# abhishekjoshi2/cuGP

Hardware: AMD Instinct MI355X
Metric: GP log-lik+grad evals/sec (N=8192, D=10) (higher is better)
Workload: dtype f64; 1 GPU; gp_loglik_grad_N8192_D10; experts=1, experts_per_gpu=1, overlap=True, full=False

## Files before the change

### cugp_amd/csrc/kernels.hip

```cpp
#include "kernels.h"

#include <hip/hip_runtime.h>
#include <hip/hip_ext.h>

#include <cassert>
#include <cstdlib>

namespace cugp {

typedef double d4 __attribute__((ext_vector_type(4)));
typedef double d2 __attribute__((ext_vector_type(2)));

template <class T>
__device__ __forceinline__ T* GP(T* p)
{
    return (T*)(__attribute__((address_space(1))) T*)(unsigned long long)p;
}

#ifdef CUGP_WGTIMES
constexpr unsigned WGT_CAP = 1u << 19;
__device__ unsigned long long g_wgt[4 * WGT_CAP];
__device__ unsigned g_wgt_n;
struct WgTimer {
    unsigned long long t0, c0, tag;
// ... 31 lines not shown
    __device__ __forceinline__ explicit LaunchStamp(unsigned long long* p_, unsigned every = 1)
        : p((p_ && (every <= 1 || blockIdx.x % every == 0 || blockIdx.x + 64 >= gridDim.x)) ? p_ : nullptr)
    {
        if (p && threadIdx.x == 0 && blockIdx.x < 64 && blockIdx.y == 0)
            __hip_atomic_fetch_min(p, (unsigned long long)__builtin_amdgcn_s_memrealtime(), __ATOMIC_RELAXED, __HIP_MEMORY_SCOPE_AGENT);
    }
    __device__ __forceinline__ ~LaunchStamp()
    {
        if (p && threadIdx.x == 0)
            __hip_atomic_fetch_max(p + STAMP_STRIDE, (unsigned long long)__builtin_amdgcn_s_memrealtime(), __ATOMIC_RELAXED, __HIP_MEMORY_SCOPE_AGENT);
    }
};

#include "cov_device.h"
#include "bcm_grad_device.h"

constexpr int BK = 16;
template <int WM> struct Geo {
    static constexpr int BT = 32 * WM;
    static constexpr int PLANE = BT * 16 + 16;
    static constexpr int OPER = (BK / 2) * PLANE;
    static constexpr int STAGE = 2 * OPER;
    static constexpr int LDS = 2 * STAGE;
};
constexpr int GEMM_LDS = Geo<4>::LDS;

constexpr int MT = 16;
constexpr int MTS = MT * (MT + 1);
constexpr int NMT = TILE / MT;
constexpr int NLT = NMT * (NMT + 1) / 2;
constexpr int POTF2_LDS = (NLT * MTS + TILE) * 8;

template <int WM>
__device__ __forceinline__ int bpos(int R)
{
    const int q = R & (16 * WM - 1);
    return (R - q) + (((q >> 5) * 2 + (q & 1)) * 16) + ((q & 31) >> 1);
}

__device__ __forceinline__ int opaque_tid()
{
    int t = threadIdx.x;
    asm volatile("" : "+v"(t));
    return t;
}

template <int WM>
__device__ __forceinline__ void tile_stage_mma(const char* __restrict__ cur, int abase, int bbase,
                                               d4 (&acc)[WM][WM])
{
    typedef Geo<WM> G;
#pragma unroll
    for (int kk = 0; kk < BK / 4; kk++) {
        double a[WM], b[WM];
#pragma unroll
        for (int m = 0; m < WM; m++) {
            a[m] = *(const double*)(cur + abase + kk * 2 * G::PLANE + m * 256);
            b[m] = *(const double*)(cur + bbase + kk * 2 * G::PLANE + m * 256);
        }
#pragma unroll
        for (int m = 0; m < WM; m++)
#pragma unroll
            for (int n = 0; n < WM; n++)
                acc[m][n] = __builtin_amdgcn_mfma_f64_16x16x4f64(a[m], b[n], acc[m][n], 0, 0, 0);
    }
}

#ifdef CUGP_TILE_STAMPS
__device__ unsigned long long g_tile_stamps[64];
__device__ int g_tile_stamp_on;
#define TILE_STAMP(i)                                                              \
    do {                                                                           \
        if (threadIdx.x == 0 && blockIdx.x == 200) {                               \
            g_tile_stamps[i] = __builtin_readcyclecounter();                       \
            g_tile_stamps[32 + i] = __builtin_amdgcn_s_memrealtime();              \
        }                                                                          \
    } while (0)
#else
#define TILE_STAMP(i)
#endif

template <bool NEGA, int WM>
__device__ __forceinline__ void tile_nt(const double* __restrict__ Ag, int lda, const double* __restrict__ Bg,
                                        int ldb, int kbeg, int kend, d4 (&acc)[WM][WM], char* smem)
{
    typedef Geo<WM> G;
    const int t = opaque_tid();
    const int lane = t & 63, wave = t >> 6;
    const int wr = wave >> 1, wc = wave & 1;

    const int srow = t >> 3, skp = t & 7;
    const double* ag = Ag + (size_t)srow * lda + 2 * skp;
    const double* bg = Bg + (size_t)srow * ldb + 2 * skp;
    d2 ra[WM], rb[WM];
    int wa[WM], wb[WM];
#pragma unroll
    for (int q = 0; q < WM; q++) {
        wa[q] = skp * G::PLANE + (srow + 32 * q) * 16;
        wb[q] = G::OPER + skp * G::PLANE + bpos<WM>(srow + 32 * q) * 16;
    }
    const int fr = lane & 15, fk = lane >> 4;
    const int abase = (fk >> 1) * G::PLANE + (wr * 16 * WM + fr) * 16 + (fk & 1) * 8;
    const int bbase = G::OPER + (fk >> 1) * G::PLANE + (wc * 16 * WM + fr) * 16 + (fk & 1) * 8;

    const int nk = (kend - kbeg) / BK;
    if (nk <= 0) return;

#pragma unroll
    for (int q = 0; q < WM; q++) {
        ra[q] = *(const d2*)(ag + (size_t)(32 * q) * lda + kbeg);
        rb[q] = *(const d2*)(bg + (size_t)(32 * q) * ldb + kbeg);
    }
#pragma unroll
    for (int q = 0; q < WM; q++) {
        *(d2*)(smem + wa[q]) = NEGA ? -ra[q] : ra[q];
        *(d2*)(smem + wb[q]) = rb[q];
    }
    __syncthreads();
#ifdef CUGP_TILE_STAMPS
    if (g_tile_stamp_on) TILE_STAMP(1);
#endif

#define CUGP_STAGE(HALF, MORE, KNEXT)                                                              \
    do {                                                                                           \
        const char* cur_ = smem + (HALF) * G::STAGE;                                               \
        char* nxt_ = smem + (1 - (HALF)) * G::STAGE;                                               \
        const bool more_ = (MORE);                                                                 \
        if (more_) {                                                                               \
            const int k_ = (KNEXT);                                                                \
            _Pragma("unroll") for (int q = 0; q < WM; q++) {                                       \
                ra[q] = *(const d2*)(ag + (size_t)(32 * q) * lda + k_);                            \
                rb[q] = *(const d2*)(bg + (size_t)(32 * q) * ldb + k_);                            \
            }                                                                                      \
        }                                                                                          \
        tile_stage_mma<WM>(cur_, abase, bbase, acc);                                               \
        if (more_) {                                                                               \
            _Pragma("unroll") for (int q = 0; q < WM; q++) {                                       \
                *(d2*)(nxt_ + wa[q]) = NEGA ? -ra[q] : ra[q];                                      \
                *(d2*)(nxt_ + wb[q]) = rb[q];                                                      \
            }                                                                                      \
        }                                                                                          \
        __syncthreads();                                                                           \
    } while (0)

    int kt = 0;
    for (; kt + 1 < nk; kt += 2) {
        CUGP_STAGE(0, true, kbeg + (kt + 1) * BK);
        CUGP_STAGE(1, kt + 2 < nk, kbeg + (kt + 2) * BK);
    }
    if (kt < nk) CUGP_STAGE(0, false, 0);
#undef CUGP_STAGE
}

template <int WM>
__device__ __forceinline__ void acc_zero(d4 (&acc)[WM][WM])
{
#pragma unroll
    for (int m = 0; m < WM; m++)
#pragma unroll
        for (int n = 0; n < WM; n++) acc[m][n] = (d4){0.0, 0.0, 0.0, 0.0};
}

#define ACC_ROW(m, r) (wr * 16 * WM + (m) * 16 + (lane >> 4) + 4 * (r))
#define ACC_COL2(np) (wc * 16 * WM + (np) * 32 + 2 * (lane & 15))

template <bool STREAM = false, int WM>
__device__ __forceinline__ void tile_load(const double* __restrict__ C, int ldc, d4 (&acc)[WM][WM])
{
    const int tid = opaque_tid();
    const int lane = tid & 63, wave = tid >> 6;
    const int wr = wave >> 1, wc = wave & 1;
#pragma unroll
    for (int m = 0; m < WM; m++)
#pragma unroll
        for (int r = 0; r < 4; r++)
#pragma unroll
            for (int np = 0; np < WM / 2; np++) {
                const d2* src = (const d2*)(C + (size_t)ACC_ROW(m, r) * ldc + ACC_COL2(np));
                const d2 v = STREAM ? __builtin_nontemporal_load(src) : *src;
                acc[m][2 * np][r] = v[0];
                acc[m][2 * np + 1][r] = v[1];
            }
}

template <bool STREAM = false, int WM>
__device__ __forceinline__ void tile_store(double* __restrict__ C, int ldc, const d4 (&acc)[WM][WM], double alpha)
{
    const int tid = opaque_tid();
    const int lane = tid & 63, wave = tid >> 6;
    const int wr = wave >> 1, wc = wave & 1;
#pragma unroll
    for (int m = 0; m < WM; m++)
#pragma unroll
        for (int r = 0; r < 4; r++)
#pragma unroll
            for (int np = 0; np < WM / 2; np++)
            {
                d2* dst = (d2*)(C + (size_t)ACC_ROW(m, r) * ldc + ACC_COL2(np));
                const d2 v = (d2){alpha * acc[m][2 * np][r], alpha * acc[m][2 * np + 1][r]};
                if (STREAM) __builtin_nontemporal_store(v, dst);
                else *dst = v;
            }
}

template <int SIGN, int WM>
__device__ __forceinline__ void tile_accum_store(double* __restrict__ C, int ldc, const d4 (&acc)[WM][WM])
{
    const int tid = opaque_tid();
    const int lane = tid & 63, wave = tid >> 6;
    const int wr = wave >> 1, wc = wave & 1;
#pragma unroll
    for (int m = 0; m < WM; m++) {
        d2 v[4][WM / 2];
#pragma unroll
        for (int r = 0; r < 4; r++)
#pragma unroll
            for (int np = 0; np < WM / 2; np++)
                v[r][np] = *(const d2*)(C + (size_t)ACC_ROW(m, r) * ldc + ACC_COL2(np));
#pragma unroll
        for (int r = 0; r < 4; r++)
#pragma unroll
            for (int np = 0; np < WM / 2; np++) {
                d2* dst = (d2*)(C + (size_t)ACC_ROW(m, r) * ldc + ACC_COL2(np));
                if (SIGN > 0) *dst = (d2){v[r][np][0] + acc[m][2 * np][r], v[r][np][1] + acc[m][2 * np + 1][r]};
                else *dst = (d2){v[r][np][0] - acc[m][2 * np][r], v[r][np][1] - acc[m][2 * np + 1][r]};
            }
    }
}

template <int WM>
__device__ __forceinline__ void tile_store_t(double* __restrict__ Ct, int ldc, const d4 (&acc)[WM][WM], double alpha,
                                             char* smem)
{
    constexpr int RH = 16 * WM, BT = 32 * WM;
    constexpr int LPC = RH / 2, CPP = 256 / LPC;
    const int t = threadIdx.x, lane = t & 63, wave = t >> 6;
    const int wr = wave >> 1, wc = wave & 1;
    double* sd = (double*)smem;
#pragma unroll
    for (int h = 0; h < 2; h++) {
        __syncthreads();
        if (wr == h) {
#pragma unroll
            for (int m = 0; m < WM; m++)
#pragma unroll
                for (int n = 0; n < WM; n++)
#pragma unroll
                    for (int r = 0; r < 4; r++) {
                        const int col = ACC_COL2(n >> 1) + (n & 1);
                        const int rr = m * 16 + (lane >> 4) + 4 * r;
                        sd[col * RH + (rr ^ ((col >> 1) & 15))] = alpha * acc[m][n][r];
                    }
        }
        __syncthreads();
        const int rr = (t % LPC) * 2;
#pragma unroll
        for (int pass = 0; pass < BT / CPP; pass++) {
            const int col = pass * CPP + t / LPC;
            const int sw = (col >> 1) & 15;
            const d2 v = (d2){sd[col * RH + (rr ^ sw)], sd[col * RH + ((rr + 1) ^ sw)]};
            *(d2*)(Ct + (size_t)col * ldc + h * RH + rr) = v;
        }
    }
}

__device__ __forceinline__ void trap_index(int idx, int wcol, int& ti, int& tj)
{
    const int head = wcol * (wcol + 1) / 2;
    if (idx < head) { tri_index(idx, ti, tj); return; }
    const int rem = idx - head;
    ti = wcol + rem / wcol;
    tj = rem % wcol;
}

template <int WM>
__device__ __forceinline__ void lauum_tile(const double* __restrict__ U, double* __restrict__ Kinv, int ld, int a, int w,
                                           int tile, int sub, char* smem)
{
    constexpr int SUB = 4 / WM, BT = 32 * WM;
    int ti, tj;
    tri_index(tile, ti, tj);
    const int si = (sub / SUB) * BT, sj = (sub % SUB) * BT;
    double* C = Kinv + (size_t)(ti * TILE + si) * ld + tj * TILE + sj;
    d4 acc[WM][WM];
    acc_zero(acc);
    tile_nt<false>(U + (size_t)(ti * TILE + si) * ld, ld, U + (size_t)(tj * TILE + sj) * ld, ld,
                   (ti < a ? a : ti) * TILE, (a + w) * TILE, acc, smem);
    if (ti < a) tile_accum_store<1>(C, ld, acc);
    else tile_store(C, ld, acc, 1.0);
}

// ... 145 lines not shown
    for (int q = 0; q < 2; q++) {
        ra[q] = *(const d2*)(ag + (size_t)(64 * q) * lda + kbeg);
        rb[q] = *(const d2*)(bg + (size_t)(64 * q) * ldb + kbeg);
    }
#pragma unroll
    for (int q = 0; q < 2; q++) {
        *(d2*)(smem + wa[q]) = NEGA ? -ra[q] : ra[q];
        *(d2*)(smem + wb[q]) = rb[q];
    }
    __syncthreads();
#define CUGP_STAGE8(HALF, MORE, KNEXT)                                                              \
    do {                                                                                            \
        const char* cur_ = smem + (HALF) * G::STAGE;                                                \
        char* nxt_ = smem + (1 - (HALF)) * G::STAGE;                                                \
        const bool more_ = (MORE);                                                                  \
        if (more_) {                                                                                \
            const int k_ = (KNEXT);                                                                 \
            _Pragma("unroll") for (int q = 0; q < 2; q++) {                                         \
                ra[q] = *(const d2*)(ag + (size_t)(64 * q) * lda + k_);                             \
                rb[q] = *(const d2*)(bg + (size_t)(64 * q) * ldb + k_);                             \
            }                                                                                       \
        }                                                                                           \
        _Pragma("unroll") for (int kk = 0; kk < BK / 4; kk++) {                                     \
            double a[2], b[4];                                                                      \
            _Pragma("unroll") for (int m = 0; m < 2; m++) a[m] = *(const double*)(cur_ + abase + kk * 2 * G::PLANE + m * 256); \
            _Pragma("unroll") for (int n = 0; n < 4; n++) b[n] = *(const double*)(cur_ + bbase + kk * 2 * G::PLANE + n * 256); \
            _Pragma("unroll") for (int m = 0; m < 2; m++)                                           \
                _Pragma("unroll") for (int n = 0; n < 4; n++)                                       \
                    acc[m][n] = __builtin_amdgcn_mfma_f64_16x16x4f64(a[m], b[n], acc[m][n], 0, 0, 0); \
        }                                                                                           \
        if (more_) {                                                                                \
            _Pragma("unroll") for (int q = 0; q < 2; q++) {                                         \
                *(d2*)(nxt_ + wa[q]) = NEGA ? -ra[q] : ra[q];                                       \
                *(d2*)(nxt_ + wb[q]) = rb[q];                                                       \
            }                                                                                       \
        }                                                                                           \
        __syncthreads();                                                                            \
    } while (0)
    int kt = 0;
    for (; kt + 1 < nk; kt += 2) {
        CUGP_STAGE8(0, true, kbeg + (kt + 1) * BK);
        CUGP_STAGE8(1, kt + 2 < nk, kbeg + (kt + 2) * BK);
    }
    if (kt < nk) CUGP_STAGE8(0, false, 0);
#undef CUGP_STAGE8
}

template <int SIGN>
__device__ __forceinline__ void tile_out8(double* __restrict__ C, int ldc, const d4 (&acc)[2][4])
{
    const int tid = opaque_tid();
    const int lane = tid & 63, wave = tid >> 6;
    const int wr = wave >> 1, wc = wave & 1;
#pragma unroll
    for (int m = 0; m < 2; m++) {
        double* const c0 = C + (size_t)(wr * 32 + m * 16 + (lane >> 4)) * ldc + wc * 64 + 2 * (lane & 15);
        d2 v[4][2];
        if (SIGN != 0) {
#pragma unroll
            for (int r = 0; r < 4; r++)
#pragma unroll
                for (int np = 0; np < 2; np++) v[r][np] = *(const d2*)(c0 + (size_t)(4 * r) * ldc + np * 32);
        }
#pragma unroll
        for (int r = 0; r < 4; r++)
#pragma unroll
            for (int np = 0; np < 2; np++) {
                d2* dst = (d2*)(c0 + (size_t)(4 * r) * ldc + np * 32);
                if (SIGN == 0) *dst = (d2){acc[m][2 * np][r], acc[m][2 * np + 1][r]};
                else if (SIGN > 0) *dst = (d2){v[r][np][0] + acc[m][2 * np][r], v[r][np][1] + acc[m][2 * np + 1][r]};
                else *dst = (d2){v[r][np][0] - acc[m][2 * np][r], v[r][np][1] - acc[m][2 * np + 1][r]};
            }
    }
}

__device__ __forceinline__ void acc_zero8(d4 (&acc)[2][4])
{
#pragma unroll
    for (int m = 0; m < 2; m++)
#pragma unroll
        for (int n = 0; n < 4; n++) acc[m][n] = (d4){0.0, 0.0, 0.0, 0.0};
}

__global__ __launch_bounds__(512, 4) void k_lauum8(const double* __restrict__ U, double* __restrict__ Kinv, int ld, int a,
                                                   int w, const ExpertPtrs* __restrict__ bt, unsigned long long* stamp)
{
    LaunchStamp stamp_(stamp);
    if (bt) { U = GP(bt[blockIdx.y].U); Kinv = GP(bt[blockIdx.y].Kinv); }
    extern __shared__ __attribute__((aligned(16))) char smem[];
    int ti, tj;
    tri_index(blockIdx.x, ti, tj);
    double* C = Kinv + (size_t)(ti * TILE) * ld + tj * TILE;
    d4 acc[2][4];
    acc_zero8(acc);
    tile_nt8<false>(U + (size_t)(ti * TILE) * ld, ld, U + (size_t)(tj * TILE) * ld, ld, (ti < a ? a : ti) * TILE,
                    (a + w) * TILE, acc, smem);
    if (ti < a) tile_out8<1>(C, ld, acc);
    else tile_out8<0>(C, ld, acc);
}

__global__ __launch_bounds__(256, 2) void k_lauum_rest(const double* __restrict__ U, double* __restrict__ Kinv, int ld,
                                                       int a, int w, int x0, const ExpertPtrs* __restrict__ bt)
{
    if (bt) { U = GP(bt[blockIdx.y].U); Kinv = GP(bt[blockIdx.y].Kinv); }
    extern __shared__ __attribute__((aligned(16))) char smem[];
    lauum_tile<2>(U, Kinv, ld, a, w, x0 + (blockIdx.x >> 2), blockIdx.x & 3, smem);
}

__global__ __launch_bounds__(512, 4) void k_trtri_border8(const double* __restrict__ L, double* __restrict__ T,
                                                          const double* __restrict__ U, int ld, int a, int w, int c0,
                                                          int c1, const ExpertPtrs* __restrict__ bt,
                                                          unsigned long long* stamp)
{
    LaunchStamp stamp_(stamp);
    if (bt) { L = GP(bt[blockIdx.y].A); T = GP(bt[blockIdx.y].T); U = GP(bt[blockIdx.y].U); }
    extern __shared__ __attribute__((aligned(16))) char smem[];
    const int tj = blockIdx.x / w, ti = a + blockIdx.x % w;
    double* W = T + (size_t)(tj * TILE) * ld + ti * TILE;
    d4 acc[2][4];
    acc_zero8(acc);
    tile_nt8<false>(U + (size_t)(tj * TILE) * ld, ld, L + (size_t)(ti * TILE) * ld, ld, (tj > c0 ? tj : c0) * TILE,
                    c1 * TILE, acc, smem);
    if (tj < c0) tile_out8<1>(W, ld, acc);
    else tile_out8<0>(W, ld, acc);
}

__global__ __launch_bounds__(256, 2) void k_trtri_border_rest(const double* __restrict__ L, double* __restrict__ T,
                                                              double* __restrict__ U, int ld, int a, int w, int c0,
                                                              int c1, int x0, const ExpertPtrs* __restrict__ bt)
{
    if (bt) { L = GP(bt[blockIdx.y].A); T = GP(bt[blockIdx.y].T); U = GP(bt[blockIdx.y].U); }
    extern __shared__ __attribute__((aligned(16))) char smem[];
    border_tile<2>(L, T, U, ld, a, w, 1, c0, c1, x0 + (blockIdx.x >> 2), blockIdx.x & 3, smem);
}

__global__ __launch_bounds__(256, 2) void k_predict_gemm(const double* __restrict__ Ks, const double* __restrict__ T,
                                                         double* __restrict__ W, int ld, int ntt64, int n64,
                                                         unsigned long long* stamp, const ExpertPtrs* __restrict__ bt)
{
    LaunchStamp stamp_(stamp);
    if (bt) {
        const size_t off = (size_t)blockIdx.y * ntt64 * 64 * ld;
        T = GP(bt[blockIdx.y].T); Ks += off; W += off;
    }
    extern __shared__ __attribute__((aligned(16))) char smem[];
    const int tt = blockIdx.x % ntt64, p = blockIdx.x / ntt64;
#pragma unroll 1
    for (int h = 0; h < 2; h++) {
        const int ti = h == 0 ? n64 - 1 - p : p;
        d4 acc[2][2];
        acc_zero(acc);
        tile_nt<false>(Ks + (size_t)tt * 64 * ld, ld, T + (size_t)ti * 64 * ld, ld, 0, (ti + 1) * 64, acc, smem);
        tile_store(W + (size_t)tt * 64 * ld + ti * 64, ld, acc, 1.0);
    }
}

__global__ __launch_bounds__(256, 2) void k_test_gemm(const double* __restrict__ A, const double* __restrict__ B,
                                                      double* __restrict__ C, int n, int k, int mt)
{
    extern __shared__ __attribute__((aligned(16))) char smem[];
    const int ti = blockIdx.x % mt, tj = blockIdx.x / mt;
    d4 acc[4][4];
    acc_zero(acc);
    tile_nt<false>(A + (size_t)ti * TILE * k, k, B + (size_t)tj * TILE * k, k, 0, k, acc, smem);
    tile_store(C + (size_t)ti * TILE * n + tj * TILE, n, acc, 1.0);
}

__global__ __launch_bounds__(256) void k_mfma_peak(double* sink, int iters)
{
    d4 acc[8];
    const double a = 1.0 + threadIdx.x * 1e-9, b = 1.0 - threadIdx.x * 1e-9;
#pragma unroll
    for (int i = 0; i < 8; i++) acc[i] = (d4){0.0, 0.0, 0.0, 0.0};
    for (int it = 0; it < iters; it++) {
#pragma unroll
        for (int i = 0; i < 8; i++) acc[i] = __builtin_amdgcn_mfma_f64_16x16x4f64(a, b, acc[i], 0, 0, 0);
    }
    double s = 0;
#pragma unroll
    for (int i = 0; i < 8; i++) s += acc[i][0] + acc[i][1] + acc[i][2] + acc[i][3];
    if (s == 12345.678) sink[blockIdx.x * 256 + threadIdx.x] = s;
}

constexpr int TRSM_TS = 68;
constexpr int TRSM_SS = 132;
constexpr int TRSM_LDS = (64 * TRSM_TS + MT * TRSM_SS + 3 * 4 * 4 * 64) * 8;

__device__ __forceinline__ void zblock_solve(const double* __restrict__ A, const double* __restrict__ d64, int ld, int kb,
                                             const double* __restrict__ w, double* __restrict__ z, double* __restrict__ sm)
{
    const int t = threadIdx.x, r = t >> 3, cg = t & 7, k0 = kb * TILE;
    double* w0 = sm;
    double* z0 = sm + 128;
    double* tt = sm + 192;
    const double* T00 = d64 + (size_t)kb * 8192;
    const double* T11 = T00 + 4096;
    const double* L10 = A + (size_t)(k0 + 64) * ld + k0;
    const int cend = (r | 15) + 1;
    double a0[8], a1[8], a2[8];
    const double wmine = t < TILE ? w[k0 + t] : 0.0;
#pragma unroll
    for (int q = 0; q < 8; q += 2) {
        const int c = cg * 8 + q;
        const d2 v0 = *(const d2*)(T00 + r * 64 + c), v1 = *(const d2*)(L10 + (size_t)r * ld + c), v2 = *(const d2*)(T11 + r * 64 + c);
        a0[q] = c < cend ? v0[0] : 0.0; a0[q + 1] = c + 1 < cend ? v0[1] : 0.0;
        a1[q] = v1[0]; a1[q + 1] = v1[1];
        a2[q] = c < cend ? v2[0] : 0.0; a2[q + 1] = c + 1 < cend ? v2[1] : 0.0;
    }
    if (t < TILE) w0[t] = wmine;
    __syncthreads();
    auto row_sum = [&](double s) {
        s += __shfl_xor(s, 1, 64);
        s += __shfl_xor(s, 2, 64);
        s += __shfl_xor(s, 4, 64);
        return s;
    };
// ... 966 lines not shown
        vec_update(A, ld, kb, kb + 1 + (bid - vec0), zv, wv);
        return;
    }
    extern __shared__ __attribute__((aligned(16))) double sm[];
    __shared__ double red[TILE + 4 * MT];
    __shared__ unsigned s_ticket;
    if (bid < NDIAGWG) {
        __builtin_amdgcn_s_setprio(3);
        WGT(wgt_, WGT_DIAGUPD, kb);
        diag_update_tile(A, ld, kb, ks, bid, sm);
#if defined(__HIP_DEVICE_COMPILE__) && !defined(__gfx950__)
#error "k_syrk_step's fence-free ticket hand-off is validated on gfx950 only: use an acq_rel ticket + agent acquire fence elsewhere"
#endif
        asm volatile("s_waitcnt vmcnt(0)" ::: "memory");
        if (threadIdx.x == 0)
            s_ticket = __hip_atomic_fetch_add(&tickets[kb], 1u, __ATOMIC_RELAXED, __HIP_MEMORY_SCOPE_AGENT);
        __syncthreads();
        if (s_ticket != NDIAGWG - 1) return;
        __builtin_amdgcn_fence(__ATOMIC_ACQUIRE, "wavefront");
        const int kn = kb + 1;
        WGT(wgt2_, WGT_POTF2, kb);
        potf2_body<true>(A + (size_t)kn * TILE * ld + kn * TILE, ld, d16 + (size_t)kn * NMT * (MT * MT),
                   d64 + (size_t)kn * 8192, logdet_part + kn, sm, red);
        return;
    }
    __builtin_amdgcn_s_setprio(1);
    WGT(wgt_, WGT_STEPTILE, kb);
    const int x = bid - NDIAGWG;
    if (x < nfull) {
        int ti, tj;
        const int xg = x & 7, xq = nfull >> 3, xr = nfull & 7;
        const int tlin = (xg < xr ? xg * (xq + 1) : xr * (xq + 1) + (xg - xr) * xq) + (x >> 3) + 1;
        trap_index((kb & 1) ? nfull + 1 - tlin : tlin, wcol, ti, tj);
        const int i0 = (kb + 1 + ti) * TILE, j0 = (kb + 1 + tj) * TILE;
        d4 acc[4][4];
        acc_zero(acc);
        tile_nt<false>(A + (size_t)i0 * ld, ld, A + (size_t)j0 * ld, ld, ks * TILE, (kb + 1) * TILE, acc, (char*)sm);
        tile_accum_store<-1>(A + (size_t)i0 * ld + j0, ld, acc);
    } else {
        int ti, tj;
        const int y = x - nfull;
        trap_index(nfull + 1 + (y >> 2), wcol, ti, tj);
        const int i0 = (kb + 1 + ti) * TILE + ((y >> 1) & 1) * 64, j0 = (kb + 1 + tj) * TILE + (y & 1) * 64;
        d4 acc[2][2];
        acc_zero(acc);
        tile_nt<false>(A + (size_t)i0 * ld, ld, A + (size_t)j0 * ld, ld, ks * TILE, (kb + 1) * TILE, acc, (char*)sm);
        tile_accum_store<-1>(A + (size_t)i0 * ld + j0, ld, acc);
    }
}

__global__ __launch_bounds__(256, 2) void k_syrk_wide(double* __restrict__ A, int ld, int k0, int kw, int ca,
                                                      int cb, int ntiles, int nfull, int rev,
                                                      const ExpertPtrs* __restrict__ bt, unsigned long long* stamp)
{
    LaunchStamp stamp_(stamp);
    if (bt) A = GP(bt[blockIdx.y].A);
    extern __shared__ __attribute__((aligned(16))) char smem[];
    __builtin_amdgcn_s_setprio(1);
    WGT(wgt_, WGT_WIDE, k0);
    if ((int)blockIdx.x >= nfull) {
        const int y = blockIdx.x - nfull;
        int ti, tj;
        trap_index(nfull + (y >> 2), cb - ca, ti, tj);
        const int i0 = (ca + ti) * TILE + ((y >> 1) & 1) * 64, j0 = (ca + tj) * TILE + (y & 1) * 64;
        d4 acc[2][2];
        acc_zero(acc);
        tile_nt<false>(A + (size_t)i0 * ld, ld, A + (size_t)j0 * ld, ld, k0 * TILE, (k0 + kw) * TILE, acc, smem);
        tile_accum_store<-1>(A + (size_t)i0 * ld + j0, ld, acc);
        return;
    }
    const int xg = blockIdx.x & 7;
    const int xq = nfull >> 3, xr = nfull & 7;
    const int tlin = (xg < xr ? xg * (xq + 1) : xr * (xq + 1) + (xg - xr) * xq) + (blockIdx.x >> 3);
    int ti, tj;
    trap_index(rev ? nfull - 1 - tlin : tlin, cb - ca, ti, tj);
    const int i0 = (ca + ti) * TILE, j0 = (ca + tj) * TILE;
    d4 acc[4][4];
    acc_zero(acc);
    tile_nt<false>(A + (size_t)i0 * ld, ld, A + (size_t)j0 * ld, ld, k0 * TILE, (k0 + kw) * TILE, acc, smem);
    tile_accum_store<-1>(A + (size_t)i0 * ld + j0, ld, acc);
}

__global__ __launch_bounds__(512, 4) void k_syrk_wide8(double* __restrict__ A, int ld, int k0, int kw, int ca, int cb,
                                                       int rev, const ExpertPtrs* __restrict__ bt,
                                                       unsigned long long* stamp)
{
    LaunchStamp stamp_(stamp);
    if (bt) A = GP(bt[blockIdx.y].A);
    extern __shared__ __attribute__((aligned(16))) char smem[];
    __builtin_amdgcn_s_setprio(1);
    const int nfull = gridDim.x;
    const int xg = blockIdx.x & 7;
    const int xq = nfull >> 3, xr = nfull & 7;
    const int tlin = (xg < xr ? xg * (xq + 1) : xr * (xq + 1) + (xg - xr) * xq) + (blockIdx.x >> 3);
    int ti, tj;
    trap_index(rev ? nfull - 1 - tlin : tlin, cb - ca, ti, tj);
    const int i0 = (ca + ti) * TILE, j0 = (ca + tj) * TILE;
    d4 acc[2][4];
    acc_zero8(acc);
    tile_nt8<false>(A + (size_t)i0 * ld, ld, A + (size_t)j0 * ld, ld, k0 * TILE, (k0 + kw) * TILE, acc, smem);
    tile_out8<-1>(A + (size_t)i0 * ld + j0, ld, acc);
}

__global__ __launch_bounds__(256, 2) void k_syrk_wide_rest(double* __restrict__ A, int ld, int k0, int kw, int ca, int cb,
                                                           int x0, const ExpertPtrs* __restrict__ bt)
{
    if (bt) A = GP(bt[blockIdx.y].A);
    extern __shared__ __attribute__((aligned(16))) char smem[];
    __builtin_amdgcn_s_setprio(1);
    const int y = blockIdx.x;
    int ti, tj;
    trap_index(x0 + (y >> 2), cb - ca, ti, tj);
    const int i0 = (ca + ti) * TILE + ((y >> 1) & 1) * 64, j0 = (ca + tj) * TILE + (y & 1) * 64;
    d4 acc[2][2];
    acc_zero(acc);
    tile_nt<false>(A + (size_t)i0 * ld, ld, A + (size_t)j0 * ld, ld, k0 * TILE, (k0 + kw) * TILE, acc, smem);
    tile_accum_store<-1>(A + (size_t)i0 * ld + j0, ld, acc);
}

__device__ __forceinline__ void trtri_diag_body(const double* __restrict__ A, int ld, int b,
                                                const double* __restrict__ d64, double* __restrict__ T,
                                                double* __restrict__ U, double* __restrict__ sm)
{
    const int t = threadIdx.x, wave = t >> 6;
    const double* Ab = A + (size_t)b * TILE * ld + b * TILE;
    const double* T00 = d64 + (size_t)b * 8192;
    const double* T11 = T00 + 4096;
    {
        const int r = t >> 4, c = t & 15;
        double v[NLT];
#pragma unroll
        for (int bi = 0; bi < NMT; bi++)
#pragma unroll
            for (int bj = 0; bj <= bi; bj++) {
                const int q = bi * (bi + 1) / 2 + bj;
                if (bi < 4) v[q] = T00[(bi * MT + r) * 64 + bj * MT + c];
                else if (bj >= 4) v[q] = T11[((bi - 4) * MT + r) * 64 + (bj - 4) * MT + c];
                else v[q] = Ab[(size_t)(bi * MT + r) * ld + bj * MT + c];
            }
#pragma unroll
        for (int q = 0; q < NLT; q++) sm[q * MTS + r * (MT + 1) + c] = v[q];
    }
    __syncthreads();
    {
        const int bj = wave;
        const d4 zero4 = (d4){0.0, 0.0, 0.0, 0.0};
        d4 w[4];
#pragma unroll
        for (int q = 0; q < 4; q++) {
            w[q] = zero4;
            for (int jp = bj; jp < 4; jp++) w[q] = micro_mma_nn(sm + mt_off(4 + q, jp), sm + mt_off(jp, bj), w[q]);
        }
        __syncthreads();
#pragma unroll
        for (int q = 0; q < 4; q++) {
            d4 x = zero4;
#pragma unroll
            for (int k = 0; k <= q; k++) x = micro_mma_acc_b(sm + mt_off(4 + q, 4 + k), w[k], x);
            asm volatile("s_waitcnt lgkmcnt(0)" ::: "memory");
            micro_store(sm + mt_off(4 + q, bj), x);
        }
    }
    __syncthreads();
    double* Tb = T + (size_t)b * TILE * ld + b * TILE;
    double* Ub = U + (size_t)b * TILE * ld + b * TILE;
#pragma unroll 8
    for (int e = t; e < TILE * TILE; e += 256) {
        const int r = e >> 7, c = e & 127, br = r >> 4, bc = c >> 4;
        Tb[(size_t)r * ld + c] = bc <= br ? sm[mt_off(br, bc) + (r & 15) * (MT + 1) + (c & 15)] : 0.0;
        Ub[(size_t)r * ld + c] = br <= bc ? sm[mt_off(bc, br) + (c & 15) * (MT + 1) + (r & 15)] : 0.0;
    }
}

__global__ __launch_bounds__(256) void k_trtri_diag(const double* __restrict__ A, int ld, int kb,
                                                    const double* __restrict__ d64, double* __restrict__ T,
                                                    double* __restrict__ U, const ExpertPtrs* __restrict__ bt)
{
    if (bt) { A = GP(bt[blockIdx.y].A); d64 = GP(bt[blockIdx.y].d64); T = GP(bt[blockIdx.y].T); U = GP(bt[blockIdx.y].U); }
    extern __shared__ __attribute__((aligned(16))) double sm[];
    WGT(wgt_, WGT_TRTRI_DIAG, kb);
    trtri_diag_body(A, ld, kb + blockIdx.x, d64, T, U, sm);
}

constexpr int TRTRI_BLOCK_LDS = TRTRI_LDS > Geo<2>::LDS ? TRTRI_LDS : Geo<2>::LDS;

__device__ __forceinline__ bool stage_barrier(unsigned* __restrict__ ctr, unsigned target, unsigned spin_cap)
{
    __shared__ int s_ok;
    asm volatile("s_waitcnt vmcnt(0)" ::: "memory");
    __syncthreads();
    if (threadIdx.x == 0) {
        __builtin_amdgcn_fence(__ATOMIC_RELEASE, "agent");
        asm volatile("s_waitcnt vmcnt(0)" ::: "memory");
        __hip_atomic_fetch_add(ctr, 1u, __ATOMIC_RELAXED, __HIP_MEMORY_SCOPE_AGENT);
        int ok = 0;
        for (unsigned spin = 0; spin < spin_cap; spin++) {
            if (__hip_atomic_load(ctr, __ATOMIC_RELAXED, __HIP_MEMORY_SCOPE_AGENT) >= target) { ok = 1; break; }
            __builtin_amdgcn_s_sleep(8);
        }
        __builtin_amdgcn_fence(__ATOMIC_ACQUIRE, "agent");
// ... 736 lines not shown
    acc_zero(acc);
    tile_tn<4>(W + ti * TILE, W + tj * TILE, ld, k0, k1, acc, smem);
    tile_store(scr + (size_t)s * pstride + (size_t)ti * TILE * ld + tj * TILE, ld, acc, 1.0);
}

thread_local hipEvent_t t_ev0 = nullptr, t_ev1 = nullptr;
thread_local unsigned long long* t_stamp = nullptr;
void time_next_launch(hipEvent_t start, hipEvent_t stop) { t_ev0 = start; t_ev1 = stop; }
void stamp_next_launch(unsigned long long* slot) { t_stamp = slot; }
bool timing_pending() { return t_ev0 != nullptr || t_stamp != nullptr; }
static inline unsigned long long* take_stamp() { unsigned long long* p = t_stamp; t_stamp = nullptr; return p; }
#define CUGP_LAUNCH(kernel, grid, block, lds, stream, ...)                                          \
    do {                                                                                            \
        if (t_ev0) {                                                                                \
            hipEvent_t e0_ = t_ev0, e1_ = t_ev1;                                                    \
            t_ev0 = t_ev1 = nullptr;                                                                \
            hipExtLaunchKernelGGL(kernel, grid, block, lds, stream, e0_, e1_, 0, __VA_ARGS__);      \
        } else {                                                                                    \
            hipLaunchKernelGGL(kernel, grid, block, lds, stream, __VA_ARGS__);                      \
        }                                                                                           \
    } while (0)

const int g_tune_init[TUNE_COUNT] = {768, 1200, 384, -1, 511, 1, 1, 1 << 20, 16, 500, 32, 1, 2100, 256, 1536, 0, 1 << 21, 1, 1, 0,
                                      1024, 64, 0};
thread_local const int* t_tune = g_tune_init;

static inline int tri_count(int n) { return n * (n + 1) / 2; }

static inline bool is_ard(const CovFn& cf)
{
    assert(!cf.ard || cf.hd);
    return cf.ard;
}

#define CUGP_COV_KERNEL(cf, stem)                                                                        \
    (is_ard(cf) ? ((cf).kind == KERNEL_MATERN32   ? stem<true, KERNEL_MATERN32>                          \
                   : (cf).kind == KERNEL_MATERN52 ? stem<true, KERNEL_MATERN52> : stem<true, KERNEL_SE>) \
                : ((cf).kind == KERNEL_MATERN32   ? stem<false, KERNEL_MATERN32>                         \
                   : (cf).kind == KERNEL_MATERN52 ? stem<false, KERNEL_MATERN52> : stem<false, KERNEL_SE>))

void launch_kbuild(const double* X, int n, int d, int npad, const CovFn& cf, double* K, bool full, hipStream_t s,
                   Batch bt, unsigned* tickets)
{
    const dim3 grid(tri_count(npad / KT), bt.count);
    hipLaunchKernelGGL(CUGP_COV_KERNEL(cf, k_build), grid, dim3(256), 0, s, X, n, d, npad, cf.h, cf.hd, K, full ? 1 : 0,
                       tickets, bt.tab, take_stamp());
}

void launch_sqdist(const double* X, int n, int d, int npad, double c, double* S, hipStream_t s)
{
    HyperScalars h{c, 0.0, 0.0};
    hipLaunchKernelGGL((k_build<false, KERNEL_SE>), dim3(tri_count(npad / KT)), dim3(256), 0, s, X, n, d, npad, h,
                       (const HyperScalars*)nullptr, S, 2, (unsigned*)nullptr, (const ExpertPtrs*)nullptr,
                       (unsigned long long*)nullptr);
}

void launch_kcross(const double* X, int n, int d, int npad, const double* Xt, int nt, int ntpad, const CovFn& cf,
                   double* Ks, hipStream_t s, Batch bt)
{
    const dim3 grid((ntpad / KT) * (npad / KT), bt.count);
    hipLaunchKernelGGL(CUGP_COV_KERNEL(cf, k_cross), grid, dim3(256), 0, s, X, n, d, npad, Xt, nt, ntpad, cf.h, Ks,
                       bt.tab, cf.hd);
}

static unsigned long long g_attr_done = 0;
static hipError_t g_attr_err = hipSuccess;
static void set_big_lds()
{
    int dev = 0;
    if (hipGetDevice(&dev) != hipSuccess || dev < 0 || dev > 63) dev = 63;
    if (g_attr_done >> dev & 1ull) return;
    hipError_t e = hipSuccess;
    auto attr = [&](const void* f, int bytes) {
        const hipError_t r = hipFuncSetAttribute(f, hipFuncAttributeMaxDynamicSharedMemorySize, bytes);
        if (r != hipSuccess && e == hipSuccess) e = r;
    };
    attr((const void*)k_potf2, POTF2_LDS);
    attr((const void*)k_syrk_step, STEP_LDS);
    attr((const void*)k_syrk_wide, GEMM_LDS);
    const void* gemm4[] = {(const void*)k_trtri_level<4>, (const void*)k_trtri_border<4>, (const void*)k_lauum<4>,
                           (const void*)k_test_gemm, (const void*)k_predict_cov<4>, (const void*)k_loo_product<4>,
                           (const void*)k_sparse_gram};
    for (const void* f : gemm4) attr(f, GEMM_LDS);
    for (const void* f : {(const void*)k_syrk_wide8, (const void*)k_lauum8, (const void*)k_trtri_border8}) attr(f, GEMM_LDS);
    attr((const void*)k_trtri_diag, TRTRI_LDS);
    attr((const void*)k_trtri_block, TRTRI_BLOCK_LDS);
    attr((const void*)k_trsm_inv64, TRSM_LDS);
    if (e != hipSuccess) { g_attr_err = e; return; }
    g_attr_done |= 1ull << dev;
}

int prepare_kernels() { set_big_lds(); return (int)g_attr_err; }

void launch_potf2(double* A, int ld, int kb, double* d16, double* d64, double* logdet_part, hipStream_t s, Batch bt)
{
    set_big_lds();
    hipLaunchKernelGGL(k_potf2, dim3(1, bt.count), dim3(256), POTF2_LDS, s, A, ld, kb, d16, d64, logdet_part, bt.tab);
}

void launch_trsm_inv64(double* A, const double* d64, int ld, int kb, int nt, hipStream_t s, Batch bt, double* zv,
                       const double* wv)
{
    const int nstrips = (nt - kb - 1) * (TILE / MT);
    if (nstrips <= 0 && !zv) return;
    set_big_lds();
    hipLaunchKernelGGL(k_trsm_inv64, dim3(nstrips + (zv ? 1 : 0), bt.count), dim3(512), TRSM_LDS, s, A, d64, ld, kb, bt.tab,
                       take_stamp(), nstrips, zv, wv);
}

void launch_trtri_diag(const double* A, int ld, int kb, int nblocks, const double* d64, double* T, double* U,
                       hipStream_t s, Batch bt)
{
    set_big_lds();
    hipLaunchKernelGGL(k_trtri_diag, dim3(nblocks, bt.count), dim3(256), TRTRI_LDS, s, A, ld, kb, d64, T, U, bt.tab);
}

int launch_trtri_block(const double* L, const double* d64, double* T, double* U, int ld, int a, int wb, unsigned* ctr,
                       double* poison, int ctr_off, hipStream_t s, Batch bt, int gcap, double* hstat)
{
    if (wb <= 0) return 0;
    set_big_lds();
    int G = wb;
    for (int sl = 1; sl < wb; sl *= 2) {
        const int items = level_tiles(wb, sl) * 4;
        if (items > G) G = items;
    }
    if (G > TRTRI_BLOCK_MAXWG) G = TRTRI_BLOCK_MAXWG;
    if (gcap >= 1 && G > gcap) G = gcap;
    CUGP_LAUNCH(k_trtri_block, dim3(G, bt.count), dim3(256), TRTRI_BLOCK_LDS, s, L, d64, T, U, ld, a, wb, ctr,
                       poison, ctr_off, (unsigned)tune(TUNE_BARRIER_SPIN), hstat, bt.tab, take_stamp());
    return G;
}

static int split_round(int tiles, int count)
{
    const int slots = 512 / (count > 0 ? count : 1) > 0 ? 512 / (count > 0 ? count : 1) : 1;
    const int rem = tiles % slots;
    if (tiles < slots || rem == 0 || rem > tune(TUNE_SPLIT_REM_MAX)) return tiles;
    return tiles - rem;
}

static inline int trap_count(int m, int wcol)
{
    return wcol >= m ? tri_count(m) : tri_count(wcol) + (m - wcol) * wcol;
}

void launch_syrk_step(double* A, int ld, int kb, int nt, double* d16, double* d64, double* logdet_part,
                      unsigned* tickets, hipStream_t s, Batch bt, int wcol, int ks, const double* zv, double* wv)
{
    const int m = nt - kb - 1;
    if (m <= 0) return;
    set_big_lds();
    if (wcol <= 0 || wcol > m) wcol = m;
    const int ntl = trap_count(m, wcol) - 1;
    int nfull = ntl;
    if (ntl >= 512 && (ntl % 512) <= tune(TUNE_SYRK_REM_MAX)) nfull = ntl - ntl % 512;
    if ((long long)ntl * bt.count * 4 <= tune(TUNE_STEP_QUARTER_MAX)) nfull = 0;
    const int vec0 = NDIAGWG + nfull + 4 * (ntl - nfull);
    const unsigned nwg = vec0 + (zv ? m : 0);
    if (ks < 0 || ks > kb) ks = kb;
    if (kb + 1 - ks > SUBPANEL_MAX) return;
    CUGP_LAUNCH(k_syrk_step, bt.tab ? dim3(bt.count, nwg) : dim3(nwg), dim3(256), STEP_LDS, s, A, ld, kb, d16,
                       d64, logdet_part, tickets, nfull, wcol, ks, bt.tab, take_stamp(), vec0, zv, wv);
}

int launch_syrk_wide(double* A, int ld, int nt, int k0, int kw, int ca, int cb, int rev, hipStream_t s, Batch bt)
{
    if (cb > nt) cb = nt;
    if (ca >= cb || kw <= 0) return 0;
    set_big_lds();
    const int ntiles = trap_count(nt - ca, cb - ca);
    const int nfull = split_round(ntiles, bt.count);
    if (tune(TUNE_WAVES8) != 0 && nfull > 0) {
        CUGP_LAUNCH(k_syrk_wide8, dim3(nfull, bt.count), dim3(512), GEMM_LDS, s, A, ld, k0, kw, ca, cb, rev, bt.tab,
                    take_stamp());
        if (ntiles > nfull)
            hipLaunchKernelGGL(k_syrk_wide_rest, dim3(4 * (ntiles - nfull), bt.count), dim3(256), Geo<2>::LDS, s, A, ld, k0,
                               kw, ca, cb, nfull, bt.tab);
        return ntiles;
    }
    CUGP_LAUNCH(k_syrk_wide, dim3(nfull + 4 * (ntiles - nfull), bt.count), dim3(256), GEMM_LDS, s, A, ld, k0, kw, ca,
                       cb, ntiles, nfull, rev, bt.tab, take_stamp());
    return ntiles;
}

int launch_trtri_level(const double* L, double* T, double* U, int ld, int nt, int s, int step, hipStream_t st,
                       Batch bt, size_t off)
{
    int tiles = 0;
    for (int a0 = 0; a0 + s < nt; a0 += 2 * s) {
        int sb = nt - (a0 + s);
        if (sb > s) sb = s;
        tiles += s * sb;
    }
    if (tiles <= 0) return 0;
    set_big_lds();
    if (tiles * bt.count <= tune(TUNE_TRTRI_WM2_MAX)) {
        CUGP_LAUNCH(k_trtri_level<2>, dim3(tiles * 4, bt.count), dim3(256), Geo<2>::LDS, st, L, T, U, ld, nt, s,
                           step, off, bt.tab, take_stamp());
        return 2;
    }
    CUGP_LAUNCH(k_trtri_level<4>, dim3(tiles, bt.count), dim3(256), GEMM_LDS, st, L, T, U, ld, nt, s, step,
                       off, bt.tab, take_stamp());
    return 4;
}

int launch_trtri_border1(const double* L, double* T, double* U, int ld, int ra, int rw, int c0, int c1,
                         hipStream_t st, Batch bt)
{
    const int tiles = c1 * rw;
    if (tiles <= 0) return 0;
    set_big_lds();
    if (tiles * bt.count <= tune(TUNE_BORDER_WM2_MAX)) {
        CUGP_LAUNCH(k_trtri_border<2>, dim3(tiles * 4, bt.count), dim3(256), Geo<2>::LDS, st, L, T, U, ld, ra, rw,
                           1, c0, c1, 0, bt.tab, take_stamp());
        return 2;
    }
    const int nfull = split_round(tiles, bt.count);
    if (tune(TUNE_WAVES8) != 0 && nfull > 0) {
        CUGP_LAUNCH(k_trtri_border8, dim3(nfull, bt.count), dim3(512), GEMM_LDS, st, L, T, U, ld, ra, rw, c0, c1, bt.tab,
                    take_stamp());
        if (tiles > nfull)
            hipLaunchKernelGGL(k_trtri_border_rest, dim3(4 * (tiles - nfull), bt.count), dim3(256), Geo<2>::LDS, st, L, T,
                               U, ld, ra, rw, c0, c1, nfull, bt.tab);
        return 4;
    }
    CUGP_LAUNCH(k_trtri_border<4>, dim3(nfull + 4 * (tiles - nfull), bt.count), dim3(256), GEMM_LDS, st, L, T,
                       U, ld, ra, rw, 1, c0, c1, nfull, bt.tab, take_stamp());
    return 4;
}

int launch_trtri_border2(const double* L, double* T, double* U, int ld, int a, int w, hipStream_t st, Batch bt)
{
    const int tiles = a * w;
    if (tiles <= 0) return 0;
    set_big_lds();
    if (tiles * bt.count <= tune(TUNE_TRTRI_WM2_MAX)) {
        CUGP_LAUNCH(k_trtri_border<2>, dim3(tiles * 4, bt.count), dim3(256), Geo<2>::LDS, st, L, T, U, ld, a, w, 2,
                           0, 0, 0, bt.tab, take_stamp());
        return 2;
    }
    const int nfull = split_round(tiles, bt.count);
    CUGP_LAUNCH(k_trtri_border<4>, dim3(nfull + 4 * (tiles - nfull), bt.count), dim3(256), GEMM_LDS, st, L, T,
                       U, ld, a, w, 2, 0, 0, nfull, bt.tab, take_stamp());
    return 4;
}

int launch_lauum(const double* U, double* Kinv, int ld, int a, int w, hipStream_t s, Batch bt)
{
    set_big_lds();
    const int tiles = tri_count(a + w);
    if (tiles * bt.count <= tune(TUNE_LAUUM_WM2_MAX)) {
        CUGP_LAUNCH(k_lauum<2>, dim3(tiles * 4, bt.count), dim3(256), Geo<2>::LDS, s, U, Kinv, ld, a, w, 0, bt.tab, take_stamp());
        return 2;
    } else {
        const int nfull = a > 0 ? split_round(tiles, bt.count) : tiles;
        if (tune(TUNE_WAVES8) != 0 && nfull > 0) {
            CUGP_LAUNCH(k_lauum8, dim3(nfull, bt.count), dim3(512), GEMM_LDS, s, U, Kinv, ld, a, w, bt.tab, take_stamp());
            if (tiles > nfull)
                hipLaunchKernelGGL(k_lauum_rest, dim3(4 * (tiles - nfull), bt.count), dim3(256), Geo<2>::LDS, s, U, Kinv, ld,
                                   a, w, nfull, bt.tab);
            return 4;
        }
        CUGP_LAUNCH(k_lauum<4>, dim3(nfull + 4 * (tiles - nfull), bt.count), dim3(256), GEMM_LDS, s, U, Kinv, ld,
                           a, w, nfull, bt.tab, take_stamp());
        return 4;
    }
}

void launch_predict_gemm(const double* Ks, const double* T, double* W, int ld, int ntt, int nt, hipStream_t s,
                         Batch bt)
{
    set_big_lds();
    CUGP_LAUNCH(k_predict_gemm, dim3(2 * ntt * nt, bt.count), dim3(256), Geo<2>::LDS, s, Ks, T, W, ld, 2 * ntt, 2 * nt,
                take_stamp(), bt.tab);
}

CovShape predict_cov_shape(int ntpad, int n)
{
    CovShape c;
    const int aim = tune(TUNE_COV_SPLIT);
    const int t128 = tri_count(ntpad / TILE);
    c.wm = (aim > 0 && 4 * t128 <= aim) ? 2 : 4;
    c.tiles = c.wm == 2 ? tri_count(ntpad / 64) : t128;
    c.kend = (n + BK - 1) / BK * BK;
    int split = aim / (c.wm == 2 ? 1 : 2) / c.tiles;
    const int kmax = c.kend / 256;
    if (split > kmax) split = kmax;
    if (split > 64) split = 64;
    const size_t pstride = (size_t)ntpad * ntpad;
    while (split > 1 && (size_t)(split - 1) * pstride * sizeof(double) > ((size_t)1 << 30)) split--;
    if (split < 1) split = 1;
    c.kstep = ((c.kend + split - 1) / split + BK - 1) / BK * BK;
    c.split = c.kstep > 0 ? (c.kend + c.kstep - 1) / c.kstep : 1;
    if (c.split < 1) c.split = 1;
    return c;
}

void launch_predict_cov(const double* W, int ld, int ntpad, const CovShape& c, double* A, double* scr, hipStream_t s)
{
    set_big_lds();
    const size_t pstride = (size_t)ntpad * ntpad;
    if (c.wm == 2)
        CUGP_LAUNCH(k_predict_cov<2>, dim3(c.tiles * c.split), dim3(256), Geo<2>::LDS, s, W, ld, c.kend, c.kstep,
                    c.split, A, scr, pstride, ntpad, take_stamp());
    else
        CUGP_LAUNCH(k_predict_cov<4>, dim3(c.tiles * c.split), dim3(256), GEMM_LDS, s, W, ld, c.kend, c.kstep,
                    c.split, A, scr, pstride, ntpad, take_stamp());
}

void launch_predict_cov_finish(const double* Xt, int nt, int d, int ntpad, const CovFn& cf, bool with_noise,
                               double jitter, double* A, const double* scr, int nscr, unsigned* tickets, hipStream_t s)
{
    const dim3 grid(tri_count(ntpad / KT));
    hipLaunchKernelGGL(CUGP_COV_KERNEL(cf, k_predict_cov_finish), grid, dim3(256), 0, s, Xt, nt, d, ntpad, cf.h,
                       with_noise ? 1 : 0, jitter, A, scr, (size_t)ntpad * ntpad, nscr, tickets, cf.hd);
}

void launch_zero_upper_diag(double* A, int ld, int nt, hipStream_t s)
{
    hipLaunchKernelGGL(k_zero_upper_diag, dim3(nt), dim3(256), 0, s, A, ld);
}

void launch_sample_finish(const double* F, int ld, const double* mean, int nt, int ns, double* out, hipStream_t s)
{
    const size_t total = (size_t)nt * ns;
    hipLaunchKernelGGL(k_sample_finish, dim3((unsigned)((total + 255) / 256)), dim3(256), 0, s, F, ld, mean, nt, ns, out);
}

void launch_predict_finish(const double* Ks, const double* W, const double* alpha, int n, int npad, int ntest,
                           HyperScalars h, double* mean, double* var, hipStream_t s, double* rows, size_t rstride,
                           int rhalf, int ntpad, Batch bt)
{
    hipLaunchKernelGGL(k_predict_finish, dim3((ntest + 3) / 4, bt.count), dim3(256), 0, s, Ks, W, alpha, n, npad,
                       ntest, h, mean, var, rows, rstride, rhalf, ntpad, bt.tab);
}

void launch_predict_grad(const double* X, int n, int d, int npad, const double* Xt, int nt, const CovFn& cf,
                         const double* Ks, const double* V, const double* alpha, double* part, size_t pstride,
                         hipStream_t s)
{
    const dim3 grid(((nt + KT - 1) / KT) * predict_grad_tiles(n));
    CUGP_LAUNCH(CUGP_COV_KERNEL(cf, k_predict_grad), grid, dim3(256), 0, s, X, n, d, npad, Xt, nt, cf.h, Ks, V, alpha, part,
                pstride, cf.hd);
// ... 315 lines not shown
```

Measured before the change: 93.60 evals/s.

## Fold 4-wave remainder tiles into the 8-wave kernels as paired half-tile workgroups

Removes the separate remainder kernels (syrk_wide_rest, lauum_rest, trtri_border_rest). The 8-wave kernels now take an nfull argument, and workgroups past nfull split into two independent 256-thread halves, each computing a 64x64 quarter tile with its own LDS region. This saves one kernel launch per call site and lets remainder tiles run in the same dispatch as the full tiles. In exchange the LDS request grows to twice the 4-wave footprint, which may reduce occupancy, and the remainder blocks no longer use the syrk_wide reversed or interleaved ordering.

```diff
diff --git a/cugp_amd/csrc/kernels.hip b/cugp_amd/csrc/kernels.hip
--- a/cugp_amd/csrc/kernels.hip
+++ b/cugp_amd/csrc/kernels.hip
@@ -137,10 +137,10 @@
 
 template <bool NEGA, int WM>
 __device__ __forceinline__ void tile_nt(const double* __restrict__ Ag, int lda, const double* __restrict__ Bg,
-                                        int ldb, int kbeg, int kend, d4 (&acc)[WM][WM], char* smem)
+                                        int ldb, int kbeg, int kend, d4 (&acc)[WM][WM], char* smem, const int half_t = -1)
 {
     typedef Geo<WM> G;
-    const int t = opaque_tid();
+    const int t = half_t >= 0 ? half_t : opaque_tid();
     const int lane = t & 63, wave = t >> 6;
     const int wr = wave >> 1, wc = wave & 1;
 
@@ -239,9 +239,10 @@
 }
 
 template <bool STREAM = false, int WM>
-__device__ __forceinline__ void tile_store(double* __restrict__ C, int ldc, const d4 (&acc)[WM][WM], double alpha)
-{
-    const int tid = opaque_tid();
+__device__ __forceinline__ void tile_store(double* __restrict__ C, int ldc, const d4 (&acc)[WM][WM], double alpha,
+                                           const int half_t = -1)
+{
+    const int tid = half_t >= 0 ? half_t : opaque_tid();
     const int lane = tid & 63, wave = tid >> 6;
     const int wr = wave >> 1, wc = wave & 1;
 #pragma unroll
@@ -259,9 +260,10 @@
 }
 
 template <int SIGN, int WM>
-__device__ __forceinline__ void tile_accum_store(double* __restrict__ C, int ldc, const d4 (&acc)[WM][WM])
-{
-    const int tid = opaque_tid();
+__device__ __forceinline__ void tile_accum_store(double* __restrict__ C, int ldc, const d4 (&acc)[WM][WM],
+                                                 const int half_t = -1)
+{
+    const int tid = half_t >= 0 ? half_t : opaque_tid();
     const int lane = tid & 63, wave = tid >> 6;
     const int wr = wave >> 1, wc = wave & 1;
 #pragma unroll
@@ -573,13 +575,45 @@
         for (int n = 0; n < 4; n++) acc[m][n] = (d4){0.0, 0.0, 0.0, 0.0};
 }
 
+constexpr int PAIR_LDS = 2 * Geo<2>::LDS;
+static_assert(PAIR_LDS >= GEMM_LDS, "the 8-wave launches ask for the pair's LDS, which must hold the whole tile's image too");
+
+struct PairHalf {
+    int tile, si, sj, t;
+    char* smem;
+    __device__ __forceinline__ PairHalf(int nfull, char* smem0)
+    {
+        const int tid = opaque_tid();
+        const int half = __builtin_amdgcn_readfirstlane(tid >> 8);
+        const int y = blockIdx.x - nfull;
+        tile = nfull + (y >> 1);
+        si = (y & 1) * 64;
+        sj = half * 64;
+        t = tid & 255;
+        smem = smem0 + half * Geo<2>::LDS;
+    }
+};
+
 __global__ __launch_bounds__(512, 4) void k_lauum8(const double* __restrict__ U, double* __restrict__ Kinv, int ld, int a,
-                                                   int w, const ExpertPtrs* __restrict__ bt, unsigned long long* stamp)
+                                                   int w, int nfull, const ExpertPtrs* __restrict__ bt,
+                                                   unsigned long long* stamp)
 {
     LaunchStamp stamp_(stamp);
     if (bt) { U = GP(bt[blockIdx.y].U); Kinv = GP(bt[blockIdx.y].Kinv); }
     extern __shared__ __attribute__((aligned(16))) char smem[];
     int ti, tj;
+    if ((int)blockIdx.x >= nfull) {
+        const PairHalf h(nfull, smem);
+        tri_index(h.tile, ti, tj);
+        double* C = Kinv + (size_t)(ti * TILE + h.si) * ld + tj * TILE + h.sj;
+        d4 acc[2][2];
+        acc_zero(acc);
+        tile_nt<false>(U + (size_t)(ti * TILE + h.si) * ld, ld, U + (size_t)(tj * TILE + h.sj) * ld, ld,
+                          (ti < a ? a : ti) * TILE, (a + w) * TILE, acc, h.smem, h.t);
+        if (ti < a) tile_accum_store<1>(C, ld, acc, h.t);
+        else tile_store(C, ld, acc, 1.0, h.t);
+        return;
+    }
     tri_index(blockIdx.x, ti, tj);
     double* C = Kinv + (size_t)(ti * TILE) * ld + tj * TILE;
     d4 acc[2][4];
@@ -590,22 +624,26 @@
     else tile_out8<0>(C, ld, acc);
 }
 
-__global__ __launch_bounds__(256, 2) void k_lauum_rest(const double* __restrict__ U, double* __restrict__ Kinv, int ld,
-                                                       int a, int w, int x0, const ExpertPtrs* __restrict__ bt)
-{
-    if (bt) { U = GP(bt[blockIdx.y].U); Kinv = GP(bt[blockIdx.y].Kinv); }
-    extern __shared__ __attribute__((aligned(16))) char smem[];
-    lauum_tile<2>(U, Kinv, ld, a, w, x0 + (blockIdx.x >> 2), blockIdx.x & 3, smem);
-}
-
 __global__ __launch_bounds__(512, 4) void k_trtri_border8(const double* __restrict__ L, double* __restrict__ T,
                                                           const double* __restrict__ U, int ld, int a, int w, int c0,
-                                                          int c1, const ExpertPtrs* __restrict__ bt,
+                                                          int c1, int nfull, const ExpertPtrs* __restrict__ bt,
                                                           unsigned long long* stamp)
 {
     LaunchStamp stamp_(stamp);
     if (bt) { L = GP(bt[blockIdx.y].A); T = GP(bt[blockIdx.y].T); U = GP(bt[blockIdx.y].U); }
     extern __shared__ __attribute__((aligned(16))) char smem[];
+    if ((int)blockIdx.x >= nfull) {
+        const PairHalf h(nfull, smem);
+        const int tj = h.tile / w, ti = a + h.tile % w;
+        double* W = T + (size_t)(tj * TILE + h.si) * ld + ti * TILE + h.sj;
+        d4 acc[2][2];
+        acc_zero(acc);
+        tile_nt<false>(U + (size_t)(tj * TILE + h.si) * ld, ld, L + (size_t)(ti * TILE + h.sj) * ld, ld,
+                          (tj > c0 ? tj : c0) * TILE, c1 * TILE, acc, h.smem, h.t);
+        if (tj < c0) tile_accum_store<1>(W, ld, acc, h.t);
+        else tile_store(W, ld, acc, 1.0, h.t);
+        return;
+    }
     const int tj = blockIdx.x / w, ti = a + blockIdx.x % w;
     double* W = T + (size_t)(tj * TILE) * ld + ti * TILE;
     d4 acc[2][4];
@@ -614,15 +652,6 @@
                     c1 * TILE, acc, smem);
     if (tj < c0) tile_out8<1>(W, ld, acc);
     else tile_out8<0>(W, ld, acc);
-}
-
-__global__ __launch_bounds__(256, 2) void k_trtri_border_rest(const double* __restrict__ L, double* __restrict__ T,
-                                                              double* __restrict__ U, int ld, int a, int w, int c0,
-                                                              int c1, int x0, const ExpertPtrs* __restrict__ bt)
-{
-    if (bt) { L = GP(bt[blockIdx.y].A); T = GP(bt[blockIdx.y].T); U = GP(bt[blockIdx.y].U); }
-    extern __shared__ __attribute__((aligned(16))) char smem[];
-    border_tile<2>(L, T, U, ld, a, w, 1, c0, c1, x0 + (blockIdx.x >> 2), blockIdx.x & 3, smem);
 }
 
 __global__ __launch_bounds__(256, 2) void k_predict_gemm(const double* __restrict__ Ks, const double* __restrict__ T,
@@ -1755,40 +1784,33 @@
 }
 
 __global__ __launch_bounds__(512, 4) void k_syrk_wide8(double* __restrict__ A, int ld, int k0, int kw, int ca, int cb,
-                                                       int rev, const ExpertPtrs* __restrict__ bt,
+                                                       int nfull, int rev, const ExpertPtrs* __restrict__ bt,
                                                        unsigned long long* stamp)
 {
     LaunchStamp stamp_(stamp);
     if (bt) A = GP(bt[blockIdx.y].A);
     extern __shared__ __attribute__((aligned(16))) char smem[];
     __builtin_amdgcn_s_setprio(1);
-    const int nfull = gridDim.x;
+    int ti, tj;
+    if ((int)blockIdx.x >= nfull) {
+        const PairHalf h(nfull, smem);
+        trap_index(h.tile, cb - ca, ti, tj);
+        const int i0 = (ca + ti) * TILE + h.si, j0 = (ca + tj) * TILE + h.sj;
+        d4 acc[2][2];
+        acc_zero(acc);
+        tile_nt<false>(A + (size_t)i0 * ld, ld, A + (size_t)j0 * ld, ld, k0 * TILE, (k0 + kw) * TILE, acc, h.smem, h.t);
+        tile_accum_store<-1>(A + (size_t)i0 * ld + j0, ld, acc, h.t);
+        return;
+    }
     const int xg = blockIdx.x & 7;
     const int xq = nfull >> 3, xr = nfull & 7;
     const int tlin = (xg < xr ? xg * (xq + 1) : xr * (xq + 1) + (xg - xr) * xq) + (blockIdx.x >> 3);
-    int ti, tj;
     trap_index(rev ? nfull - 1 - tlin : tlin, cb - ca, ti, tj);
     const int i0 = (ca + ti) * TILE, j0 = (ca + tj) * TILE;
     d4 acc[2][4];
     acc_zero8(acc);
     tile_nt8<false>(A + (size_t)i0 * ld, ld, A + (size_t)j0 * ld, ld, k0 * TILE, (k0 + kw) * TILE, acc, smem);
     tile_out8<-1>(A + (size_t)i0 * ld + j0, ld, acc);
-}
-
-__global__ __launch_bounds__(256, 2) void k_syrk_wide_rest(double* __restrict__ A, int ld, int k0, int kw, int ca, int cb,
-                                                           int x0, const ExpertPtrs* __restrict__ bt)
-{
-    if (bt) A = GP(bt[blockIdx.y].A);
-    extern __shared__ __attribute__((aligned(16))) char smem[];
-    __builtin_amdgcn_s_setprio(1);
-    const int y = blockIdx.x;
-    int ti, tj;
-    trap_index(x0 + (y >> 2), cb - ca, ti, tj);
-    const int i0 = (ca + ti) * TILE + ((y >> 1) & 1) * 64, j0 = (ca + tj) * TILE + (y & 1) * 64;
-    d4 acc[2][2];
-    acc_zero(acc);
-    tile_nt<false>(A + (size_t)i0 * ld, ld, A + (size_t)j0 * ld, ld, k0 * TILE, (k0 + kw) * TILE, acc, smem);
-    tile_accum_store<-1>(A + (size_t)i0 * ld + j0, ld, acc);
 }
 
 __device__ __forceinline__ void trtri_diag_body(const double* __restrict__ A, int ld, int b,
@@ -2691,7 +2713,7 @@
                            (const void*)k_test_gemm, (const void*)k_predict_cov<4>, (const void*)k_loo_product<4>,
                            (const void*)k_sparse_gram};
     for (const void* f : gemm4) attr(f, GEMM_LDS);
-    for (const void* f : {(const void*)k_syrk_wide8, (const void*)k_lauum8, (const void*)k_trtri_border8}) attr(f, GEMM_LDS);
+    for (const void* f : {(const void*)k_syrk_wide8, (const void*)k_lauum8, (const void*)k_trtri_border8}) attr(f, PAIR_LDS);
     attr((const void*)k_trtri_diag, TRTRI_LDS);
     attr((const void*)k_trtri_block, TRTRI_BLOCK_LDS);
     attr((const void*)k_trsm_inv64, TRSM_LDS);
@@ -2781,11 +2803,8 @@
     const int ntiles = trap_count(nt - ca, cb - ca);
     const int nfull = split_round(ntiles, bt.count);
     if (tune(TUNE_WAVES8) != 0 && nfull > 0) {
-        CUGP_LAUNCH(k_syrk_wide8, dim3(nfull, bt.count), dim3(512), GEMM_LDS, s, A, ld, k0, kw, ca, cb, rev, bt.tab,
-                    take_stamp());
-        if (ntiles > nfull)
-            hipLaunchKernelGGL(k_syrk_wide_rest, dim3(4 * (ntiles - nfull), bt.count), dim3(256), Geo<2>::LDS, s, A, ld, k0,
-                               kw, ca, cb, nfull, bt.tab);
+        CUGP_LAUNCH(k_syrk_wide8, dim3(nfull + 2 * (ntiles - nfull), bt.count), dim3(512), PAIR_LDS, s, A, ld, k0, kw, ca, cb,
+                    nfull, rev, bt.tab, take_stamp());
         return ntiles;
     }
     CUGP_LAUNCH(k_syrk_wide, dim3(nfull + 4 * (ntiles - nfull), bt.count), dim3(256), GEMM_LDS, s, A, ld, k0, kw, ca,
@@ -2827,11 +2846,8 @@
     }
     const int nfull = split_round(tiles, bt.count);
     if (tune(TUNE_WAVES8) != 0 && nfull > 0) {
-        CUGP_LAUNCH(k_trtri_border8, dim3(nfull, bt.count), dim3(512), GEMM_LDS, st, L, T, U, ld, ra, rw, c0, c1, bt.tab,
-                    take_stamp());
-        if (tiles > nfull)
-            hipLaunchKernelGGL(k_trtri_border_rest, dim3(4 * (tiles - nfull), bt.count), dim3(256), Geo<2>::LDS, st, L, T,
-                               U, ld, ra, rw, c0, c1, nfull, bt.tab);
+        CUGP_LAUNCH(k_trtri_border8, dim3(nfull + 2 * (tiles - nfull), bt.count), dim3(512), PAIR_LDS, st, L, T, U, ld, ra, rw,
+                    c0, c1, nfull, bt.tab, take_stamp());
         return 4;
     }
     CUGP_LAUNCH(k_trtri_border<4>, dim3(nfull + 4 * (tiles - nfull), bt.count), dim3(256), GEMM_LDS, st, L, T,
@@ -2865,10 +2881,8 @@
     } else {
         const int nfull = a > 0 ? split_round(tiles, bt.count) : tiles;
         if (tune(TUNE_WAVES8) != 0 && nfull > 0) {
-            CUGP_LAUNCH(k_lauum8, dim3(nfull, bt.count), dim3(512), GEMM_LDS, s, U, Kinv, ld, a, w, bt.tab, take_stamp());
-            if (tiles > nfull)
-                hipLaunchKernelGGL(k_lauum_rest, dim3(4 * (tiles - nfull), bt.count), dim3(256), Geo<2>::LDS, s, U, Kinv, ld,
-                                   a, w, nfull, bt.tab);
+            CUGP_LAUNCH(k_lauum8, dim3(nfull + 2 * (tiles - nfull), bt.count), dim3(512), PAIR_LDS, s, U, Kinv, ld, a, w, nfull,
+                        bt.tab, take_stamp());
             return 4;
         }
         CUGP_LAUNCH(k_lauum<4>, dim3(nfull + 4 * (tiles - nfull), bt.count), dim3(256), GEMM_LDS, s, U, Kinv, ld,
```

Result: no change. 93.20 evals/s (-0.4%).
